# tensorlink-lab/tensorlink

Measured on AMD Instinct MI355X. Metric: output tokens/sec (Qwen2.5-7B serving, PP sharded), higher is better.
Workload: dtype bf16; 1 GPU; model=Qwen/Qwen2.5-7B-Instruct, global_batch=256, seq_len=512, parallelism=pp1, micro_batches=4

## Files before the change

tensorlink_amd/models/dense.py:

```python

from __future__ import annotations

import dataclasses

import math
from typing import List, Optional

import torch
import torch.nn as nn

from tensorlink_amd import ops
from tensorlink_amd.models.configs import ModelConfig


class KVCache:

    def __init__(self, n_layers: int, batch: int, max_seq: int, config,
                 device, dtype=torch.bfloat16):
        self.k = [torch.zeros(batch, config.num_key_value_heads, max_seq,
                              config.head_dim, device=device, dtype=dtype)
                  for _ in range(n_layers)]
        self.v = [torch.zeros_like(self.k[0]) for _ in range(n_layers)]
        self.seq_lens = torch.zeros(batch, device=device, dtype=torch.int32)
        self.max_seq = max_seq
# ... 79 lines not shown
        eps = self.config.rms_norm_eps
        fuse = fuse and kv_cache is not None and not training
        if fuse and not self.use_qk_norm:
            qkv = _project(self.qkv_proj, x, allow_bias=True)
        else:
            qkv = self.qkv_proj(x)
        flat_pos = positions.reshape(-1)

        if training or kv_cache is None:
            q, k, v = self._split_qkv(qkv, B, S)
            if self.use_qk_norm:
                q = ops.rmsnorm(q.contiguous(), self.q_norm.to(q.dtype), eps)
                k = ops.rmsnorm(k.contiguous(), self.k_norm.to(k.dtype), eps)
            if training:
                q2, k2 = ops.apply_rope(q.reshape(B * S, self.n_heads, -1),
                                        k.reshape(B * S, self.n_kv, -1),
                                        flat_pos, self.inv_freq)
                q = q2.view(B, S, self.n_heads, -1)
                k = k2.view(B, S, self.n_kv, -1)
                out = ops.attention_train(q, k, v, causal=True,
                                          scale=self.scale)
            else:
                q = q.contiguous()
                k = k.contiguous()
                ops.apply_rope_(q.view(B * S, self.n_heads, -1),
                                k.view(B * S, self.n_kv, -1), flat_pos,
                                self.inv_freq)
                out = ops.attention_prefill(q, k, v.contiguous(),
                                            causal=True, scale=self.scale)
            return self.o_proj(out.reshape(B, S, -1))

        table = getattr(kv_cache, "table", None)
        if self.use_qk_norm:
            q, k, v = self._split_qkv(qkv, B, S)
            q = ops.rmsnorm(q.contiguous(), self.q_norm.to(q.dtype), eps)
            k = ops.rmsnorm(k.contiguous(), self.k_norm.to(k.dtype), eps)
            qkv = torch.cat([q.reshape(B, S, -1), k.reshape(B, S, -1),
                             v.reshape(B, S, -1)], dim=-1)
        if not isinstance(qkv, ops.Partials):
            qkv = qkv.reshape(B * S, -1)
        q = ops.rope_append_(qkv, kv_cache.k[layer_idx],
                             kv_cache.v[layer_idx], flat_pos, self.inv_freq,
                             S, self.n_heads, self.n_kv, block_table=table)
        q = q.view(B, S, self.n_heads, self.head_dim)
        if S == 1 and fuse:
            out = ops.attention_decode(
                q, kv_cache.k[layer_idx], kv_cache.v[layer_idx],
                kv_cache.seq_lens, scale=self.scale, block_table=table,
                len_add=1)
        elif S == 1:
            out = ops.attention_decode(
                q, kv_cache.k[layer_idx], kv_cache.v[layer_idx],
                kv_cache.seq_lens + 1, scale=self.scale, block_table=table)
        else:
            if B > 1:
                assert int(kv_cache.seq_lens.min()) == \
                    int(kv_cache.seq_lens.max()), \
                    "ragged cached prefill needs per-row q_off"
            off = int(kv_cache.seq_lens.max())
            kv_len = off + S
            if table is None:
                k_attn = kv_cache.k[layer_idx][:, :, :kv_len].permute(
                    0, 2, 1, 3).contiguous()
                v_attn = kv_cache.v[layer_idx][:, :, :kv_len].permute(
                    0, 2, 1, 3).contiguous()
            else:
                k_attn, v_attn = kv_cache.gather_contiguous(layer_idx, kv_len)
            out = ops.attention_prefill(q, k_attn, v_attn, causal=True,
                                        scale=self.scale, q_off=off)
        if fuse:
            return _project(self.o_proj, out.reshape(B, S, -1))
        return self.o_proj(out.reshape(B, S, -1))


class MLP(nn.Module):
    def __init__(self, config: ModelConfig):
        super().__init__()
        h, i = config.hidden_size, config.intermediate_size
        self.inter = i
        self.gate_up_proj = TLLinear(h, 2 * i, bias=False)
        self.down_proj = TLLinear(i, h, bias=False)

    def forward(self, x, fuse: bool = False):
        gu = self.gate_up_proj(x)
        if torch.is_grad_enabled() and gu.requires_grad:
            gate, up = gu.split([self.inter, self.inter], dim=-1)
            return self.down_proj(ops.swiglu(gate.contiguous(),
                                             up.contiguous()))
        if fuse:
            return _project(self.down_proj, ops.swiglu_fused(gu))
        return self.down_proj(ops.swiglu_fused(gu))


class MoEMLP(nn.Module):

    def __init__(self, config: ModelConfig):
        super().__init__()
        h, i = config.hidden_size, config.intermediate_size
        self.num_experts = config.num_local_experts
        self.top_k = config.num_experts_per_tok
        self.gate = nn.Linear(h, self.num_experts, bias=False)
        expert_cfg = (config if config.expert_intermediate_size == i
                      else dataclasses.replace(
                          config,
                          intermediate_size=config.expert_intermediate_size))
        self.experts = nn.ModuleList([MLP(expert_cfg)
                                      for _ in range(self.num_experts)])

    def _fused_kind(self):
        from tensorlink_amd.models.quant import Fp4Linear, Fp8Linear
        e0 = self.experts[0]
        if isinstance(e0.gate_up_proj, Fp8Linear):
            return "fp8"
        if isinstance(e0.gate_up_proj, Fp4Linear):
            for e in self.experts:
                for p in (e.gate_up_proj, e.down_proj):
                    if not (isinstance(p, Fp4Linear) and p.bias is None
                            and p.out_features % 64 == 0
                            and p.in_features % 128 == 0):
                        return None
            return "fp4"
        if isinstance(e0.gate_up_proj, nn.Linear) \
                and e0.gate_up_proj.bias is None:
            return "bf16"
        return None

    def _tables(self, dev, kind):
        wname = {"fp8": "weight_fp8", "fp4": "packed"}.get(kind, "weight")
        sname = {"fp8": "scale", "fp4": "exponents"}.get(kind)
        gus = [getattr(e.gate_up_proj, wname) for e in self.experts]
        key = (str(dev), kind, gus[0].data_ptr())
        if getattr(self, "_tbl_key", None) != key:
            downs = [getattr(e.down_proj, wname) for e in self.experts]

            def mk(ts):
                if kind == "fp4":
                    assert all(t.is_contiguous()
                               and t.data_ptr() % 16 == 0 for t in ts), \
                        "fp4 expert tensors must be contiguous and " \
                        "16-byte aligned"
                return torch.tensor([t.data_ptr() for t in ts],
                                    dtype=torch.int64, device=dev)
            self._gu_ptrs = mk(gus)
            self._down_ptrs = mk(downs)
            if sname is not None:
                self._gu_scales = mk([getattr(e.gate_up_proj, sname)
                                      for e in self.experts])
                self._down_scales = mk([getattr(e.down_proj, sname)
                                        for e in self.experts])
            else:
                self._gu_scales = self._down_scales = None
            self._tbl_key = key
        return (self._gu_ptrs, self._down_ptrs, self._gu_scales,
                self._down_scales)

    def _fused_forward(self, flat, rw, idx, kind=None):
        C = ops._require_ext()
        kind = kind if kind is not None else self._fused_kind()
        E, k = self.num_experts, self.top_k
        T, H = flat.shape
        P = T * k
        dev = flat.device
        gu_p, down_p, gu_s, down_s = self._tables(dev, kind)
        fi = idx.reshape(-1)
        order = fi.argsort(stable=True)
        counts = torch.zeros(E, device=dev, dtype=torch.long)
        counts.scatter_add_(0, fi, torch.ones_like(fi))
        seg = torch.zeros(E + 1, device=dev, dtype=torch.int32)
        seg[1:] = counts.cumsum(0)
        pair_tok = (order // k).to(torch.int32)
        Ie = self.experts[0].inter
        if kind == "fp4":
            gu = ops.mxfp4_moe_gemm(flat.contiguous(), pair_tok, seg, gu_p,
                                    gu_s, 2 * Ie)
# ... 186 lines not shown
```

tensorlink_amd/ops/__init__.py:

```python

from __future__ import annotations

import math
from typing import Optional

import torch

from tensorlink_amd.ops import reference as ref

_C = None
_IMPORT_ERROR: Optional[BaseException] = None
try:
    from tensorlink_amd import _C
except Exception as e:
    _IMPORT_ERROR = e


def extension_loaded() -> bool:
    return _C is not None


def _require_ext():
    if _C is None:
        raise RuntimeError(
# ... 234 lines not shown
        ctx.causal = causal
        ctx.scale = scale
        return out

    @staticmethod
    def backward(ctx, dout):
        C = _require_ext()
        q, k, v, out, lse = ctx.saved_tensors
        delta = (dout.float() * out.float()).sum(-1)
        delta = delta.permute(0, 2, 1).contiguous()
        dq, dk, dv = C.attn_bwd(q.contiguous(), k.contiguous(),
                                v.contiguous(), dout.contiguous(), lse,
                                delta, ctx.scale, ctx.causal)
        return dq, dk, dv, None, None


def attention_train(q, k, v, causal: bool = True,
                    scale: Optional[float] = None) -> torch.Tensor:
    B, S, Hq, D = q.shape
    Hkv = k.shape[2]
    if scale is None:
        scale = 1.0 / math.sqrt(D)
    if (q.is_cuda and q.dtype == torch.bfloat16 and _C is not None
            and D in (64, 128) and k.shape[1] == S):
        return _FlashAttnFn.apply(q, k, v, causal, scale)
    qt = q.transpose(1, 2)
    kt = k.transpose(1, 2)
    vt = v.transpose(1, 2)
    try:
        out = torch.nn.functional.scaled_dot_product_attention(
            qt, kt, vt, is_causal=causal, scale=scale, enable_gqa=True)
    except (TypeError, RuntimeError):
        rep = Hq // Hkv
        out = torch.nn.functional.scaled_dot_product_attention(
            qt, kt.repeat_interleave(rep, dim=1),
            vt.repeat_interleave(rep, dim=1), is_causal=causal, scale=scale)
    return out.transpose(1, 2)


def attention_decode(q, k_cache, v_cache, seq_lens,
                     scale: Optional[float] = None, n_split: int = 0,
                     block_table: Optional[torch.Tensor] = None,
                     len_add: int = 0) -> torch.Tensor:
    squeeze = q.dim() == 4
    if squeeze:
        q3 = q.squeeze(1)
    else:
        q3 = q
    scale = scale if scale is not None else 1.0 / math.sqrt(q3.shape[-1])
    if not _on_gpu(q3):
        if len_add:
            seq_lens = seq_lens + len_add
        if block_table is not None:
            B = q3.shape[0]
            L = int(seq_lens.max())
            np_ = (L + 127) // 128
            idx = block_table[:, :np_].long()
            kc = k_cache[idx].permute(0, 1, 3, 2, 4)
            vc = v_cache[idx].permute(0, 1, 3, 2, 4)
            kc = kc.reshape(B, np_ * 128, *kc.shape[3:])[:, :L]
            vc = vc.reshape(B, np_ * 128, *vc.shape[3:])[:, :L]
            out = ref.attention_decode(q3.unsqueeze(1), kc, vc, seq_lens,
                                       scale)
        else:
            out = ref.attention_decode(q3.unsqueeze(1),
                                       k_cache.permute(0, 2, 1, 3),
                                       v_cache.permute(0, 2, 1, 3),
                                       seq_lens, scale)
        return out if squeeze else out.squeeze(1)
    out = _require_ext().decode_attn(
        q3.contiguous(), k_cache, v_cache, seq_lens.int(), scale, n_split,
        block_table.int() if block_table is not None else None, len_add)
    return out.unsqueeze(1) if squeeze else out


import os as _os

GEMM_M_MAX = int(_os.environ.get("TL_GEMM_M_MAX", "512"))

gemm_dispatch_count = 0


_LIB_CLASSES = frozenset(
    c for c in _os.environ.get("TL_GEMM_LIB_CLASSES",
                               "gateup").split(",") if c)


def _gemm_class(N: int, K: int) -> str:
    if N >= 65536:
        return "wide"
    if N >= 16384:
        return "gateup"
    if K >= 8192:
        return "deepk"
    return "narrow"


def _use_tl_gemm(M: int, N: int, K: int) -> bool:
    return (K % 32 == 0 and N % 64 == 0 and M <= GEMM_M_MAX
            and _gemm_class(N, K) not in _LIB_CLASSES)


def linear(x: torch.Tensor, weight: torch.Tensor,
           bias: Optional[torch.Tensor] = None) -> torch.Tensor:
    global gemm_dispatch_count
    if (x.is_cuda and not torch.is_grad_enabled()
            and x.dtype == torch.bfloat16
            and not _os.environ.get("TL_NO_SKINNY")):
        K = x.shape[-1]
        M = x.numel() // K
        N = weight.shape[0]
        if _use_tl_gemm(M, N, K):
            gemm_dispatch_count += 1
            return _require_ext().skinny_gemm(
                x.contiguous(), weight,
                bias.to(torch.bfloat16) if bias is not None else None)
    return torch.nn.functional.linear(x, weight, bias)


def decode_fusion_enabled() -> bool:
    return not _os.environ.get("TL_NO_DECODE_FUSION")


def linear_partials(x: torch.Tensor, weight: torch.Tensor,
                    bias: Optional[torch.Tensor] = None):
    global gemm_dispatch_count
    if (x.is_cuda and not torch.is_grad_enabled()
            and x.dtype == torch.bfloat16
            and not _os.environ.get("TL_NO_SKINNY")):
        K = x.shape[-1]
        M = x.numel() // K
        N = weight.shape[0]
        if _use_tl_gemm(M, N, K):
            gemm_dispatch_count += 1
            b = bias.to(torch.bfloat16) if bias is not None else None
            out = _require_ext().skinny_gemm_partials(x.contiguous(),
                                                      weight, b)
            if out.dtype == torch.float32:
                return Partials(out, b)
            return out
    return linear(x, weight, bias)


mxfp4_dispatch_count = 0


def _use_mxfp4_gemm(M: int, N: int, K: int) -> bool:
    return (N > 0 and N % 64 == 0 and K > 0 and K % 128 == 0
            and 1 <= M <= min(GEMM_M_MAX, 512))


def mxfp4_linear(x: torch.Tensor, packed: torch.Tensor,
                 exponents: torch.Tensor,
                 bias: Optional[torch.Tensor] = None) -> torch.Tensor:
    global mxfp4_dispatch_count
    if not _on_gpu(x):
        return ref.mxfp4_linear(x, packed, exponents, bias)
    K = x.shape[-1]
    M = x.numel() // K if K else 0
    N = packed.shape[0]
    if (x.dtype == torch.bfloat16 and _C is not None
            and _use_mxfp4_gemm(M, N, K)):
        mxfp4_dispatch_count += 1
        return _C.mxfp4_gemm(
            x.contiguous(), packed.contiguous(), exponents.contiguous(),
            bias.to(torch.bfloat16).contiguous()
            if bias is not None else None)
    w = ref.dequantize_mxfp4(packed, exponents, dtype=torch.bfloat16)
    return torch.nn.functional.linear(
        x, w.to(x.dtype), bias.to(x.dtype) if bias is not None else None)


mxfp4_moe_dispatch_count = 0


def mxfp4_moe_gemm(x: torch.Tensor, tok_idx: Optional[torch.Tensor],
                   seg_off: torch.Tensor, p_ptrs: torch.Tensor,
                   e_ptrs: torch.Tensor, N: int) -> torch.Tensor:
    global mxfp4_moe_dispatch_count
    out = _require_ext().mxfp4_moe_gemm(x, tok_idx, seg_off, p_ptrs, e_ptrs,
                                        N)
    mxfp4_moe_dispatch_count += 1
    return out


def adamw_(param: torch.Tensor, grad: torch.Tensor, exp_avg: torch.Tensor,
           exp_avg_sq: torch.Tensor, *, lr: float, beta1: float = 0.9,
           beta2: float = 0.999, eps: float = 1e-8,
           weight_decay: float = 0.0, step: int = 1) -> None:
    if not _on_gpu(param):
        ref.adamw_step(param, grad, exp_avg, exp_avg_sq, lr=lr, beta1=beta1,
                       beta2=beta2, eps=eps, weight_decay=weight_decay,
                       step=step)
        return
    _require_ext().adamw_(param, grad.contiguous(), exp_avg, exp_avg_sq, lr,
                          beta1, beta2, eps, weight_decay, step)


def _splitmix64(x: int) -> int:
    x = (x + 0x9E3779B97F4A7C15) & (2 ** 64 - 1)
# ... 37 lines not shown
```

tensorlink_amd/ops/csrc/bindings.cpp:

```cpp

#include <torch/extension.h>

#include <c10/hip/HIPStream.h>
#include <hip/hip_runtime.h>

extern "C" {
void tl_rmsnorm_fwd(const void* x, const void* residual, const void* w,
                    void* y, void* r_out, void* rstd, int64_t N, int H,
                    float eps, hipStream_t stream);
void tl_rmsnorm_add_fwd(const void* x, const void* residual, const void* w,
                        void* y, void* r_out, int64_t N, int H, float eps,
                        int n_split, int mode, hipStream_t stream);
void tl_rmsnorm_bwd(const void* dy, const void* x, const void* w,
                    const void* rstd, void* dx, void* dw, void* dw_partial,
                    int n_blocks, int64_t N, int H, hipStream_t stream);
void tl_rope(void* q, void* k, const void* positions, const void* inv_freq,
             int64_t T, int Hq, int Hkv, int D, float sign,
             hipStream_t stream);
void tl_swiglu_fwd(const void* gate, const void* up, void* out, int64_t n,
                   hipStream_t stream);
void tl_swiglu_bwd(const void* dout, const void* gate, const void* up,
                   void* dgate, void* dup, int64_t n, hipStream_t stream);
void tl_adamw(void* param, const void* grad, void* m, void* v, int64_t n,
              int is_bf16, float lr, double beta1, double beta2, float eps,
              float weight_decay, int step, hipStream_t stream);
void tl_decode_attn(const void* q, const void* k_cache, const void* v_cache,
                    const void* seq_lens, void* out, int B, int Hq, int Hkv,
                    int Smax, int D, float scale, int len_add,
                    hipStream_t stream);
void tl_prefill_attn(const void* q, const void* k, const void* v, void* out,
                     int B, int Sq, int Skv, int q_off, int Hq, int Hkv,
                     int D, float scale, int causal, hipStream_t stream);
void tl_rope_append(const void* qkv, const void* bias, void* q_out,
                    void* k_cache, void* v_cache, const void* positions,
                    const void* inv_freq, const void* block_table,
                    int64_t T, int row_stride, int S, int Hq, int Hkv,
                    int D, int Smax, int bt_stride, int n_split,
                    int inv_bf16, hipStream_t stream);
void tl_swiglu_fused(const void* gu, void* out, int64_t N, int I,
                     hipStream_t stream);
void tl_decode_attn_mfma(const void* q, const void* k_cache,
                         const void* v_cache, const void* seq_lens,
                         const void* block_table, void* out,
                         void* partial, void* partial_ml, int B, int Hq,
                         int Hkv, int Smax, int D, float scale, int n_split,
                         int bt_stride, int per_row, int len_add,
                         hipStream_t stream);
void tl_skinny_gemm(const void* x, const void* w, const void* bias,
                    void* out, void* partial, int M, int N, int K,
                    int n_split, hipStream_t stream);
void tl_gemm_tiled(const void* x, const void* w, const void* bias, void* out,
                   void* partial, int M, int N, int K, int n_split,
                   hipStream_t stream);
void tl_skinny_gemm_partials(const void* x, const void* w, const void* bias,
                             void* out, void* partial, int M, int N, int K,
                             int n_split, hipStream_t stream);
void tl_gemm_tiled_partials(const void* x, const void* w, const void* bias,
                            void* out, void* partial, int M, int N, int K,
                            int n_split, hipStream_t stream);
void tl_sample(const void* logits, const void* temps, const void* top_ps,
               const void* top_ks, const void* pres, const void* freqs,
               void* counts, const void* seeds, const void* ctr, void* out,
               uint64_t seed_base, int B, int V, hipStream_t stream);
void tl_bump_counter(void* ctr, hipStream_t stream);
void tl_moe_gemm(const void* x, const void* tok_idx, const void* seg_off,
                 const void* w_ptrs, const void* s_ptrs, void* out, int E,
                 int N, int K, int fp8, hipStream_t stream);
void tl_mxfp4_gemm(const void* x, const void* packed, const void* exps,
                   const void* bias, void* out, void* partial, int M, int N,
                   int K, int n_split, hipStream_t stream);
void tl_mxfp4_moe_gemm(const void* x, const void* tok_idx,
                       const void* seg_off, const void* p_ptrs,
                       const void* e_ptrs, void* out, void* partial, int T,
                       int P, int E, int N, int K, int n_split,
                       hipStream_t stream);
void tl_prefill_attn_lse(const void* q, const void* k, const void* v,
                         void* out, void* lse, int B, int Sq, int Skv,
                         int q_off, int Hq, int Hkv, int D, float scale,
                         int causal, hipStream_t stream);
void tl_attn_bwd(const void* q, const void* k, const void* v,
                 const void* dout, const void* lse, const void* delta,
                 void* dq, void* dk, void* dv, int B, int S, int Hq,
                 int Hkv, int D, float scale, int causal,
                 hipStream_t stream);
}

namespace {

hipStream_t cur_stream() {
  return c10::hip::getCurrentHIPStream().stream();
}

int tl_split_for_len(int L) {
  int ns = 1;
  while (ns < 16 && L > 1024 * ns) ns <<= 1;
  return ns;
}

#define CHECK_IN(t, d)                                              \
  TORCH_CHECK((t).is_cuda(), #t " must be on GPU");                 \
  TORCH_CHECK((t).is_contiguous(), #t " must be contiguous");       \
  TORCH_CHECK((t).scalar_type() == (d), #t " wrong dtype")

using torch::Tensor;

std::vector<Tensor> rmsnorm_fwd(Tensor x, c10::optional<Tensor> residual,
                                Tensor w, double eps, bool save_rstd) {
  CHECK_IN(x, torch::kBFloat16);
  CHECK_IN(w, torch::kBFloat16);
  const int H = x.size(-1);
  TORCH_CHECK(H % 8 == 0, "H must be divisible by 8");
  TORCH_CHECK(H <= 16384, "rmsnorm supports H <= 16384");
  const int64_t N = x.numel() / H;
  auto y = torch::empty_like(x);
  Tensor rstd, r_out;
  if (save_rstd) rstd = torch::empty({N}, x.options().dtype(torch::kFloat));
  const void* res_ptr = nullptr;
  void* rout_ptr = nullptr;
  if (residual.has_value()) {
    CHECK_IN(residual.value(), torch::kBFloat16);
    r_out = torch::empty_like(x);
    res_ptr = residual->data_ptr();
    rout_ptr = r_out.data_ptr();
  }
  tl_rmsnorm_fwd(x.data_ptr(), res_ptr, w.data_ptr(), y.data_ptr(), rout_ptr,
                 save_rstd ? rstd.data_ptr() : nullptr, N, H, (float)eps,
                 cur_stream());
  std::vector<Tensor> outs = {y};
  if (residual.has_value()) outs.push_back(r_out);
  if (save_rstd) outs.push_back(rstd);
  return outs;
}

std::vector<Tensor> rmsnorm_add_fwd(Tensor x, Tensor residual,
                                    c10::optional<Tensor> w, double eps,
                                    int64_t mode) {
  CHECK_IN(residual, torch::kBFloat16);
  TORCH_CHECK(mode >= 1 && mode <= 3, "mode must be 1, 2 or 3");
  const int H = residual.size(-1);
  TORCH_CHECK(H % 8 == 0, "H must be divisible by 8");
  TORCH_CHECK(H <= 16384, "rmsnorm supports H <= 16384");
  const int64_t N = residual.numel() / H;
// ... 281 lines not shown
}

static int gemm_split_target() {
  static int t = [] {
    const char* e = getenv("TL_GEMM_SPLIT_TARGET");
    return e ? atoi(e) : 256;
  }();
  return t;
}

static int gemm_n_split(int N, int K) {
  if (N >= 65536) {
    int n_split = 1;
    while (((N + 255) / 256) * n_split < gemm_split_target() &&
           n_split < 16 && (K / 64) / (n_split * 2) >= 16)
      n_split <<= 1;
    return n_split;
  }
  int n_split = 1;
  while ((N / 64) * n_split < gemm_split_target() && n_split < 8 &&
         (K / 32) / (n_split * 2) >= 2)
    n_split <<= 1;
  return n_split;
}

Tensor skinny_gemm(Tensor x, Tensor w, c10::optional<Tensor> bias) {
  CHECK_IN(x, torch::kBFloat16);
  CHECK_IN(w, torch::kBFloat16);
  const int K = x.size(-1);
  const int64_t M = x.numel() / K;
  const int N = w.size(0);
  TORCH_CHECK(w.size(1) == K, "K mismatch");
  TORCH_CHECK(K % 32 == 0 && N % 64 == 0, "unsupported shape");
  auto sizes = x.sizes().vec();
  sizes.back() = N;
  auto out = torch::empty(sizes, x.options());
  const void* bp = nullptr;
  if (bias.has_value()) {
    CHECK_IN(bias.value(), torch::kBFloat16);
    bp = bias->data_ptr();
  }
  const int n_split = gemm_n_split(N, K);
  Tensor partial;
  void* pp = nullptr;
  if (n_split > 1) {
    partial = torch::empty({(int64_t)n_split * M * N},
                           x.options().dtype(torch::kFloat));
    pp = partial.data_ptr();
  }
  if (M <= 64)
    tl_skinny_gemm(x.data_ptr(), w.data_ptr(), bp, out.data_ptr(), pp,
                   (int)M, N, K, n_split, cur_stream());
  else
    tl_gemm_tiled(x.data_ptr(), w.data_ptr(), bp, out.data_ptr(), pp,
                  (int)M, N, K, n_split, cur_stream());
  return out;
}

Tensor skinny_gemm_partials(Tensor x, Tensor w, c10::optional<Tensor> bias) {
  CHECK_IN(x, torch::kBFloat16);
  CHECK_IN(w, torch::kBFloat16);
  const int K = x.size(-1);
  const int64_t M = x.numel() / K;
  const int N = w.size(0);
  TORCH_CHECK(w.size(1) == K, "K mismatch");
  TORCH_CHECK(K % 32 == 0 && N % 64 == 0, "unsupported shape");
  const int n_split = gemm_n_split(N, K);
  if (n_split == 1) return skinny_gemm(x, w, bias);
  auto sizes = x.sizes().vec();
  sizes.back() = N;
  sizes.insert(sizes.begin(), n_split);
  auto partial = torch::empty(sizes, x.options().dtype(torch::kFloat));
  if (M <= 64)
    tl_skinny_gemm_partials(x.data_ptr(), w.data_ptr(), nullptr, nullptr,
                            partial.data_ptr(), (int)M, N, K, n_split,
                            cur_stream());
  else
    tl_gemm_tiled_partials(x.data_ptr(), w.data_ptr(), nullptr, nullptr,
                           partial.data_ptr(), (int)M, N, K, n_split,
                           cur_stream());
  return partial;
}

static int mxfp4_split_for_blocks(int blocks, int K) {
  int n_split = 1;
  while (blocks * n_split < 256 && n_split < 8 &&
         (K / 128) / (n_split * 2) >= 2)
    n_split <<= 1;
  return n_split;
}

static int mxfp4_n_split(int N, int K) {
  return mxfp4_split_for_blocks(N / 64, K);
}

static int mxfp4_moe_n_split(int N, int K, int E) {
  return mxfp4_split_for_blocks((N / 64) * E, K);
}

int64_t mxfp4_n_split_py(int64_t N, int64_t K) {
  TORCH_CHECK(N > 0 && K > 0 && N % 64 == 0 && K % 128 == 0,
              "unsupported shape");
  return mxfp4_n_split((int)N, (int)K);
}

int64_t mxfp4_moe_n_split_py(int64_t N, int64_t K, int64_t E) {
  TORCH_CHECK(N > 0 && K > 0 && E > 0 && N % 64 == 0 && K % 128 == 0,
              "unsupported shape");
  return mxfp4_moe_n_split((int)N, (int)K, (int)E);
}

Tensor mxfp4_gemm(Tensor x, Tensor packed, Tensor exponents,
                  c10::optional<Tensor> bias) {
  CHECK_IN(x, torch::kBFloat16);
  CHECK_IN(packed, torch::kByte);
  CHECK_IN(exponents, torch::kChar);
  TORCH_CHECK(packed.dim() == 2 && exponents.dim() == 2,
              "packed / exponents must be 2-D");
  TORCH_CHECK(x.dim() >= 1, "x must have a K dimension");
  const int64_t K = x.size(-1);
  const int64_t N = packed.size(0);
  TORCH_CHECK(K > 0 && N > 0 && N % 64 == 0 && K % 128 == 0,
              "unsupported shape: need N % 64 == 0 and K % 128 == 0");
  TORCH_CHECK(packed.size(1) * 2 == K, "packed must be [N, K/2]");
  TORCH_CHECK(exponents.size(0) == N && exponents.size(1) * 32 == K,
              "exponents must be [N, K/32]");
  const int64_t M = x.numel() / K;
  TORCH_CHECK(M >= 1 && M <= 512, "mxfp4_gemm supports 1 <= M <= 512");
  TORCH_CHECK(packed.device() == x.device() &&
                  exponents.device() == x.device(),
              "operands must share a device");
  auto sizes = x.sizes().vec();
  sizes.back() = N;
  auto out = torch::empty(sizes, x.options());
  const void* bp = nullptr;
  if (bias.has_value()) {
    CHECK_IN(bias.value(), torch::kBFloat16);
    TORCH_CHECK(bias->numel() == N, "bias must be [N]");
    bp = bias->data_ptr();
  }
  const int n_split = mxfp4_n_split((int)N, (int)K);
  Tensor partial;
  void* pp = nullptr;
  if (n_split > 1) {
    partial = torch::empty({(int64_t)n_split * M * N},
                           x.options().dtype(torch::kFloat));
    pp = partial.data_ptr();
  }
  tl_mxfp4_gemm(x.data_ptr(), packed.data_ptr(), exponents.data_ptr(), bp,
                out.data_ptr(), pp, (int)M, (int)N, (int)K, n_split,
                cur_stream());
  return out;
}

Tensor sample_tokens(Tensor logits, Tensor temps, Tensor top_ps,
                     Tensor top_ks, Tensor pres, Tensor freqs,
                     c10::optional<Tensor> counts,
                     c10::optional<Tensor> seeds,
                     c10::optional<Tensor> counter, int64_t seed_base) {
  CHECK_IN(logits, torch::kBFloat16);
  CHECK_IN(temps, torch::kFloat);
  CHECK_IN(top_ps, torch::kFloat);
  CHECK_IN(top_ks, torch::kInt);
  CHECK_IN(pres, torch::kFloat);
  CHECK_IN(freqs, torch::kFloat);
  const int B = logits.size(0);
// ... 40 lines not shown
  const void* ti = nullptr;
  int64_t P;
  if (tok_idx.has_value()) {
    CHECK_IN(tok_idx.value(), torch::kInt);
    ti = tok_idx->data_ptr();
    P = tok_idx->size(0);
  } else {
    P = x.size(0);
  }
  const void* sp = nullptr;
  if (fp8) {
    TORCH_CHECK(s_ptrs.has_value(), "fp8 needs scale pointers");
    CHECK_IN(s_ptrs.value(), torch::kLong);
    sp = s_ptrs->data_ptr();
  }
  auto out = torch::empty({P, N}, x.options());
  tl_moe_gemm(x.data_ptr(), ti, seg_off.data_ptr(), w_ptrs.data_ptr(), sp,
              out.data_ptr(), E, (int)N, K, fp8 ? 1 : 0, cur_stream());
  return out;
}

Tensor mxfp4_moe_gemm(Tensor x, c10::optional<Tensor> tok_idx,
                      Tensor seg_off, Tensor p_ptrs, Tensor e_ptrs,
                      int64_t N, int64_t n_split_override) {
  CHECK_IN(x, torch::kBFloat16);
  CHECK_IN(seg_off, torch::kInt);
  CHECK_IN(p_ptrs, torch::kLong);
  CHECK_IN(e_ptrs, torch::kLong);
  TORCH_CHECK(x.dim() == 2, "x must be [T, K]");
  const int64_t T = x.size(0);
  const int64_t K = x.size(1);
  TORCH_CHECK(K > 0 && N > 0 && N % 64 == 0 && K % 128 == 0,
              "unsupported shape: need N % 64 == 0 and K % 128 == 0");
  TORCH_CHECK(p_ptrs.dim() == 1 && e_ptrs.dim() == 1 &&
                  p_ptrs.size(0) == e_ptrs.size(0),
              "pointer tables must both be [E]");
  const int64_t E = p_ptrs.size(0);
  TORCH_CHECK(E >= 1 && E <= 65535, "need 1 <= E <= 65535");
  TORCH_CHECK(seg_off.dim() == 1 && seg_off.size(0) == E + 1,
              "seg_off must be [E+1]");
  TORCH_CHECK(seg_off.device() == x.device() &&
                  p_ptrs.device() == x.device() &&
                  e_ptrs.device() == x.device(),
              "operands must share a device");
  const void* ti = nullptr;
  int64_t P = T;
  if (tok_idx.has_value()) {
    CHECK_IN(tok_idx.value(), torch::kInt);
    TORCH_CHECK(tok_idx->dim() == 1, "tok_idx must be [P]");
    TORCH_CHECK(tok_idx->device() == x.device(),
                "operands must share a device");
    ti = tok_idx->data_ptr();
    P = tok_idx->size(0);
  }
  TORCH_CHECK(P * N < (int64_t)1 << 31 && T * K < (int64_t)1 << 40,
              "mxfp4_moe_gemm: call too large");
  auto out = torch::empty({P, N}, x.options());
  if (P == 0) return out;
  TORCH_CHECK(T >= 1, "x has no rows");
  const int n_split = n_split_override > 0
                          ? (int)n_split_override
                          : mxfp4_moe_n_split((int)N, (int)K, (int)E);
  TORCH_CHECK(n_split >= 1 && n_split <= 8, "bad split count");
  Tensor partial;
  void* pp = nullptr;
  if (n_split > 1) {
    partial = torch::empty({(int64_t)n_split * P * N},
                           x.options().dtype(torch::kFloat));
    pp = partial.data_ptr();
  }
  tl_mxfp4_moe_gemm(x.data_ptr(), ti, seg_off.data_ptr(), p_ptrs.data_ptr(),
                    e_ptrs.data_ptr(), out.data_ptr(), pp, (int)T, (int)P,
                    (int)E, (int)N, (int)K, n_split, cur_stream());
  return out;
}

}

PYBIND11_MODULE(TORCH_EXTENSION_NAME, mod) {
  mod.def("rope_append_", &rope_append_,
          "fused RoPE + KV-cache append from fused-QKV rows");
  mod.def("swiglu_fused", &swiglu_fused, "silu-mul on fused [.,2I] rows");
  mod.def("skinny_gemm", &skinny_gemm, "decode-M GEMM: x @ W^T + bias");
  mod.def("skinny_gemm_partials", &skinny_gemm_partials,
          "decode-M GEMM handing out its fp32 split-K partials");
  mod.def("rmsnorm_add_fwd", &rmsnorm_add_fwd,
          "residual add + RMSNorm from bf16 or split-K partials");
  mod.def("rmsnorm_fwd", &rmsnorm_fwd, "fused RMSNorm fwd (+residual)");
  mod.def("rmsnorm_bwd", &rmsnorm_bwd, "RMSNorm bwd");
  mod.def("rope_", &rope_, "in-place RoPE apply");
  mod.def("swiglu_fwd", &swiglu_fwd, "silu(gate)*up");
  mod.def("swiglu_bwd", &swiglu_bwd, "SwiGLU bwd");
  mod.def("adamw_", &adamw_, "fused AdamW step");
  mod.def("decode_attn", &decode_attn, "GQA decode attention over KV cache");
  mod.def("prefill_attn", &prefill_attn, "causal GQA prefill attention");
  mod.def("sample_tokens", &sample_tokens,
          "fused penalties/temperature/top-k/top-p sampling, one block/row");
  mod.def("bump_sample_counter", &bump_sample_counter,
          "advance the graph-safe sampling RNG counter");
  mod.def("moe_gemm", &moe_gemm,
          "grouped expert GEMM over expert-sorted pair rows");
  mod.def("mxfp4_gemm", &mxfp4_gemm,
          "weight-only MXFP4 GEMM: x @ dequant(packed, exponents)^T + bias");
  mod.def("mxfp4_n_split", &mxfp4_n_split_py,
          "split-K count of mxfp4_gemm for (N, K)");
  mod.def("mxfp4_moe_gemm", &mxfp4_moe_gemm,
          "grouped MXFP4 expert GEMM over expert-sorted pair rows",
          pybind11::arg("x"), pybind11::arg("tok_idx"),
          pybind11::arg("seg_off"), pybind11::arg("p_ptrs"),
          pybind11::arg("e_ptrs"), pybind11::arg("N"),
          pybind11::arg("n_split_override") = 0);
  mod.def("mxfp4_moe_n_split", &mxfp4_moe_n_split_py,
          "split-K count of mxfp4_moe_gemm for (N, K, E)");
  mod.def("prefill_attn_lse", &prefill_attn_lse,
          "causal GQA prefill attention returning (out, logsumexp)");
  mod.def("attn_bwd", &attn_bwd,
          "flash-attention backward: (dq, dk, dv) from saved lse/delta");
}
```

tensorlink_amd/ops/csrc/swiglu.hip:

```cpp

#include "common.hpp"

namespace {

constexpr int BLOCK = 256;

DEVINLINE float silu(float x) { return x / (1.f + __expf(-x)); }

__global__ __launch_bounds__(BLOCK) void swiglu_fwd_kernel(
    const bf16* __restrict__ gate, const bf16* __restrict__ up,
    bf16* __restrict__ out, int64_t n8) {
  const int64_t i = ((int64_t)blockIdx.x * BLOCK + threadIdx.x);
  if (i >= n8) return;
  bf16x8 g = reinterpret_cast<const bf16x8*>(gate)[i];
  bf16x8 u = reinterpret_cast<const bf16x8*>(up)[i];
  bf16x8 o;
#pragma unroll
  for (int j = 0; j < 8; ++j)
    o.v[j] = f2bf(silu(bf2f(g.v[j])) * bf2f(u.v[j]));
  reinterpret_cast<bf16x8*>(out)[i] = o;
}

__global__ __launch_bounds__(BLOCK) void swiglu_fused_kernel(
    const bf16* __restrict__ gu, bf16* __restrict__ out, int64_t N, int I) {
  const int64_t i = ((int64_t)blockIdx.x * BLOCK + threadIdx.x) * 8;
  if (i >= N * (int64_t)I) return;
  const int64_t r = i / I;
  const int64_t c = i - r * I;
  const bf16x8 g = *reinterpret_cast<const bf16x8*>(gu + r * 2 * I + c);
  const bf16x8 u = *reinterpret_cast<const bf16x8*>(gu + r * 2 * I + I + c);
  bf16x8 o;
#pragma unroll
  for (int j = 0; j < 8; ++j)
    o.v[j] = f2bf(silu(bf2f(g.v[j])) * bf2f(u.v[j]));
  *reinterpret_cast<bf16x8*>(out + r * I + c) = o;
}

__global__ __launch_bounds__(BLOCK) void swiglu_bwd_kernel(
    const bf16* __restrict__ dout, const bf16* __restrict__ gate,
    const bf16* __restrict__ up, bf16* __restrict__ dgate,
    bf16* __restrict__ dup, int64_t n8) {
  const int64_t i = ((int64_t)blockIdx.x * BLOCK + threadIdx.x);
  if (i >= n8) return;
  bf16x8 dO = reinterpret_cast<const bf16x8*>(dout)[i];
  bf16x8 g = reinterpret_cast<const bf16x8*>(gate)[i];
  bf16x8 u = reinterpret_cast<const bf16x8*>(up)[i];
  bf16x8 dg, du;
#pragma unroll
  for (int j = 0; j < 8; ++j) {
    const float gv = bf2f(g.v[j]);
    const float sig = 1.f / (1.f + __expf(-gv));
    const float si = gv * sig;
    const float dsilu = sig * (1.f + gv * (1.f - sig));
    const float dov = bf2f(dO.v[j]);
    dg.v[j] = f2bf(dov * bf2f(u.v[j]) * dsilu);
    du.v[j] = f2bf(dov * si);
  }
  reinterpret_cast<bf16x8*>(dgate)[i] = dg;
  reinterpret_cast<bf16x8*>(dup)[i] = du;
}

}

extern "C" {

void tl_swiglu_fwd(const void* gate, const void* up, void* out, int64_t n,
                   hipStream_t stream) {
  const int64_t n8 = n / 8;
  dim3 grid((uint32_t)cdiv(n8, BLOCK)), block(BLOCK);
  hipLaunchKernelGGL(swiglu_fwd_kernel, grid, block, 0, stream,
                     (const bf16*)gate, (const bf16*)up, (bf16*)out, n8);
}

void tl_swiglu_fused(const void* gu, void* out, int64_t N, int I,
                     hipStream_t stream) {
  const int64_t work = N * (int64_t)I / 8;
  dim3 grid((uint32_t)((work + BLOCK - 1) / BLOCK)), block(BLOCK);
  hipLaunchKernelGGL(swiglu_fused_kernel, grid, block, 0, stream,
                     (const bf16*)gu, (bf16*)out, N, I);
}

void tl_swiglu_bwd(const void* dout, const void* gate, const void* up,
                   void* dgate, void* dup, int64_t n, hipStream_t stream) {
  const int64_t n8 = n / 8;
  dim3 grid((uint32_t)cdiv(n8, BLOCK)), block(BLOCK);
  hipLaunchKernelGGL(swiglu_bwd_kernel, grid, block, 0, stream,
                     (const bf16*)dout, (const bf16*)gate, (const bf16*)up,
                     (bf16*)dgate, (bf16*)dup, n8);
}

}
```

Before: 13800 tokens/s.

## Add column-balanced gate_up GEMM with fused SwiGLU epilogue

```diff
diff --git a/tensorlink_amd/models/dense.py b/tensorlink_amd/models/dense.py
--- a/tensorlink_amd/models/dense.py
+++ b/tensorlink_amd/models/dense.py
@@ -185,14 +185,19 @@
         self.down_proj = TLLinear(i, h, bias=False)
 
     def forward(self, x, fuse: bool = False):
-        gu = self.gate_up_proj(x)
-        if torch.is_grad_enabled() and gu.requires_grad:
-            gate, up = gu.split([self.inter, self.inter], dim=-1)
-            return self.down_proj(ops.swiglu(gate.contiguous(),
-                                             up.contiguous()))
+        if (type(self.gate_up_proj) is TLLinear and not
+                torch.is_grad_enabled()):
+            act = ops.gate_up_swiglu(x, self.gate_up_proj.weight)
+        else:
+            gu = self.gate_up_proj(x)
+            if torch.is_grad_enabled() and gu.requires_grad:
+                gate, up = gu.split([self.inter, self.inter], dim=-1)
+                return self.down_proj(ops.swiglu(gate.contiguous(),
+                                                 up.contiguous()))
+            act = ops.swiglu_fused(gu)
         if fuse:
-            return _project(self.down_proj, ops.swiglu_fused(gu))
-        return self.down_proj(ops.swiglu_fused(gu))
+            return _project(self.down_proj, act)
+        return self.down_proj(act)
 
 
 class MoEMLP(nn.Module):
diff --git a/tensorlink_amd/ops/__init__.py b/tensorlink_amd/ops/__init__.py
--- a/tensorlink_amd/ops/__init__.py
+++ b/tensorlink_amd/ops/__init__.py
@@ -340,8 +340,7 @@
 
 
 _LIB_CLASSES = frozenset(
-    c for c in _os.environ.get("TL_GEMM_LIB_CLASSES",
-                               "gateup").split(",") if c)
+    c for c in _os.environ.get("TL_GEMM_LIB_CLASSES", "").split(",") if c)
 
 
 def _gemm_class(N: int, K: int) -> str:
@@ -359,21 +358,53 @@
             and _gemm_class(N, K) not in _LIB_CLASSES)
 
 
+_n_split_cache = {}
+
+
+def _use_colbal(M: int, N: int, K: int) -> bool:
+    if not (65 <= M and _use_tl_gemm(M, N, K)
+            and _gemm_class(N, K) == "gateup"
+            and not _os.environ.get("TL_NO_COLBAL")):
+        return False
+    ns = _n_split_cache.get((N, K))
+    if ns is None:
+        ns = _n_split_cache[(N, K)] = _require_ext().gemm_n_split(N, K)
+    return ns == 1
+
+
+def _family_input(x: torch.Tensor) -> bool:
+    return (x.is_cuda and not torch.is_grad_enabled()
+            and x.dtype == torch.bfloat16
+            and not _os.environ.get("TL_NO_SKINNY"))
+
+
 def linear(x: torch.Tensor, weight: torch.Tensor,
            bias: Optional[torch.Tensor] = None) -> torch.Tensor:
     global gemm_dispatch_count
-    if (x.is_cuda and not torch.is_grad_enabled()
-            and x.dtype == torch.bfloat16
-            and not _os.environ.get("TL_NO_SKINNY")):
+    if _family_input(x):
         K = x.shape[-1]
         M = x.numel() // K
         N = weight.shape[0]
+        if bias is None and _use_colbal(M, N, K):
+            gemm_dispatch_count += 1
+            return _require_ext().gemm_colbal(x.contiguous(), weight)
         if _use_tl_gemm(M, N, K):
             gemm_dispatch_count += 1
             return _require_ext().skinny_gemm(
                 x.contiguous(), weight,
                 bias.to(torch.bfloat16) if bias is not None else None)
     return torch.nn.functional.linear(x, weight, bias)
+
+
+def gate_up_swiglu(x: torch.Tensor, weight: torch.Tensor) -> torch.Tensor:
+    global gemm_dispatch_count
+    if _family_input(x) and not _os.environ.get("TL_NO_GATEUP_FUSION"):
+        K = x.shape[-1]
+        M = x.numel() // K
+        if _use_colbal(M, weight.shape[0], K):
+            gemm_dispatch_count += 1
+            return _require_ext().gemm_colbal_swiglu(x.contiguous(), weight)
+    return swiglu_fused(linear(x, weight))
 
 
 def decode_fusion_enabled() -> bool:
diff --git a/tensorlink_amd/ops/csrc/bindings.cpp b/tensorlink_amd/ops/csrc/bindings.cpp
--- a/tensorlink_amd/ops/csrc/bindings.cpp
+++ b/tensorlink_amd/ops/csrc/bindings.cpp
@@ -58,6 +58,8 @@
 void tl_gemm_tiled_partials(const void* x, const void* w, const void* bias,
                             void* out, void* partial, int M, int N, int K,
                             int n_split, hipStream_t stream);
+void tl_gemm_colbal(const void* x, const void* w, void* out, int M, int N,
+                    int K, int n_blocks, int fused, hipStream_t stream);
 void tl_sample(const void* logits, const void* temps, const void* top_ps,
                const void* top_ks, const void* pres, const void* freqs,
                void* counts, const void* seeds, const void* ctr, void* out,
@@ -505,6 +507,52 @@
   return partial;
 }
 
+static int device_cu_count(int dev) {
+  static int cus[64] = {0};
+  TORCH_CHECK(dev >= 0 && dev < 64, "device index out of range");
+  if (cus[dev] == 0) {
+    int n = 0;
+    TORCH_CHECK(hipDeviceGetAttribute(
+                    &n, hipDeviceAttributeMultiprocessorCount, dev) ==
+                        hipSuccess && n > 0,
+                "cannot read the CU count");
+    cus[dev] = n;
+  }
+  return cus[dev];
+}
+
+static Tensor gemm_colbal_impl(Tensor x, Tensor w, int64_t n_blocks,
+                               bool fused) {
+  CHECK_IN(x, torch::kBFloat16);
+  CHECK_IN(w, torch::kBFloat16);
+  const int K = x.size(-1);
+  const int64_t M = x.numel() / K;
+  const int N = w.size(0);
+  TORCH_CHECK(w.dim() == 2 && w.size(1) == K, "K mismatch");
+  TORCH_CHECK(K % 32 == 0 && K >= 32 && M >= 1 && M < (1 << 24),
+              "unsupported shape");
+  TORCH_CHECK(N % (fused ? 32 : 16) == 0 && N > 0, "unsupported width");
+  TORCH_CHECK(gemm_n_split(N, K) == 1,
+              "gemm_colbal serves only shapes the policy does not split");
+  if (n_blocks <= 0) n_blocks = device_cu_count(x.get_device());
+  TORCH_CHECK(n_blocks <= 65535, "n_blocks too large");
+  const int NO = fused ? N / 2 : N;
+  auto sizes = x.sizes().vec();
+  sizes.back() = NO;
+  auto out = torch::empty(sizes, x.options());
+  tl_gemm_colbal(x.data_ptr(), w.data_ptr(), out.data_ptr(), (int)M, NO, K,
+                 (int)n_blocks, fused ? 1 : 0, cur_stream());
+  return out;
+}
+
+Tensor gemm_colbal(Tensor x, Tensor w, int64_t n_blocks) {
+  return gemm_colbal_impl(x, w, n_blocks, false);
+}
+
+Tensor gemm_colbal_swiglu(Tensor x, Tensor w_gate_up, int64_t n_blocks) {
+  return gemm_colbal_impl(x, w_gate_up, n_blocks, true);
+}
+
 static int mxfp4_split_for_blocks(int blocks, int K) {
   int n_split = 1;
   while (blocks * n_split < 256 && n_split < 8 &&
@@ -711,6 +759,14 @@
           "fused RoPE + KV-cache append from fused-QKV rows");
   mod.def("swiglu_fused", &swiglu_fused, "silu-mul on fused [.,2I] rows");
   mod.def("skinny_gemm", &skinny_gemm, "decode-M GEMM: x @ W^T + bias");
+  mod.def("gemm_n_split", &gemm_n_split,
+          "split-K count the GEMM family's (N,K)-only policy gives");
+  mod.def("gemm_colbal", &gemm_colbal,
+          "column-balanced one-pass GEMM: x @ W^T (n_split == 1 shapes)",
+          py::arg("x"), py::arg("w"), py::arg("n_blocks") = 0);
+  mod.def("gemm_colbal_swiglu", &gemm_colbal_swiglu,
+          "column-balanced gate_up GEMM with SwiGLU on the accumulators",
+          py::arg("x"), py::arg("w_gate_up"), py::arg("n_blocks") = 0);
   mod.def("skinny_gemm_partials", &skinny_gemm_partials,
           "decode-M GEMM handing out its fp32 split-K partials");
   mod.def("rmsnorm_add_fwd", &rmsnorm_add_fwd,
diff --git a/tensorlink_amd/ops/csrc/gemm_colbal.hip b/tensorlink_amd/ops/csrc/gemm_colbal.hip
--- /dev/null
+++ b/tensorlink_amd/ops/csrc/gemm_colbal.hip
@@ -0,0 +1,241 @@
+
+#include "common.hpp"
+#include "swiglu_common.hpp"
+
+namespace {
+
+using f32x4 = __attribute__((ext_vector_type(4))) float;
+typedef __bf16 bf16x8_t __attribute__((ext_vector_type(8)));
+
+constexpr int CB_BM = 256;
+constexpr int CB_SLOTS = 10;
+constexpr int CB_ROWS = CB_BM + CB_SLOTS * 16;
+constexpr int CB_STAGES = 3;
+constexpr int CB_STAGE_ELEMS = CB_ROWS * 64;
+constexpr int CB_CPAD = 168;
+
+template <int N>
+DEVINLINE void cb_waitcnt_vm() {
+  asm volatile("s_waitcnt vmcnt(%0)" ::"n"(N) : "memory");
+}
+
+template <int FUSED>
+__global__ __launch_bounds__(512, 1) void gemm_colbal_kernel(
+    const bf16* __restrict__ x,
+    const bf16* __restrict__ w,
+    bf16* __restrict__ out,
+    int M, int NO, int K) {
+  const int tid = threadIdx.x;
+  const int lane = tid & 63;
+  const int wave = __builtin_amdgcn_readfirstlane(tid >> 6);
+  const int col = lane & 15;
+  const int quad = lane >> 4;
+  const int wm = wave >> 1;
+  const int wn = wave & 1;
+  const int l8 = lane >> 3, c8 = lane & 7;
+  const int m_base = blockIdx.z * CB_BM;
+
+  constexpr int SPT = FUSED ? 2 : 1;
+  constexpr int MAXT = CB_SLOTS / SPT;
+
+  const int T = NO / 16, G = gridDim.x, b = blockIdx.x;
+  const int q = T / G, r = T % G;
+  const int cnt = q + (b < r ? 1 : 0);
+  const int start = b * q + min(b, r);
+  if (cnt == 0) return;
+  const int n_sub = (cnt + MAXT - 1) / MAXT;
+
+  __shared__ bf16 lds[CB_STAGES * CB_STAGE_ELEMS];
+
+  const bool active = m_base + wm * 64 < M;
+  const int n_full = K / 64, n_chunks = (K + 63) / 64;
+
+  for (int s = 0; s < n_sub; ++s) {
+    const int sq = cnt / n_sub, sr = cnt % n_sub;
+    const int t0 = start + s * sq + min(s, sr);
+    const int tc = sq + (s < sr ? 1 : 0);
+
+    int64_t xoff[4], woff[3];
+#pragma unroll
+    for (int g = 0; g < 4; ++g) {
+      const int row = (wave * 4 + g) * 8 + l8;
+      xoff[g] = (int64_t)min(m_base + row, M - 1) * K;
+    }
+#pragma unroll
+    for (int g = 0; g < 3; ++g) {
+      const int wchunk = min(wave + g * 8, 19);
+      const int slot = wchunk >> 1;
+      const int half = FUSED ? (slot >= MAXT ? 1 : 0) : 0;
+      const int tile = t0 + min(slot - half * MAXT, tc - 1);
+      woff[g] = ((int64_t)half * NO + tile * 16 + (wchunk & 1) * 8 + l8) * K;
+    }
+
+    auto stage = [&](int bufi, int k0) {
+      bf16* sbase = lds + bufi * CB_STAGE_ELEMS;
+      const int kc = min(k0 + (c8 ^ l8) * 8, K - 8);
+#pragma unroll
+      for (int g = 0; g < 4; ++g) {
+        auto gsrc = (const __attribute__((address_space(1))) void*)(
+            x + xoff[g] + kc);
+        auto ldst = (__attribute__((address_space(3))) void*)(
+            sbase + (wave * 4 + g) * 8 * 64);
+        __builtin_amdgcn_global_load_lds(gsrc, ldst, 16, 0, 0);
+      }
+#pragma unroll
+      for (int g = 0; g < 3; ++g) {
+        if (g == 2 && wave >= 4) break;
+        auto gsrc = (const __attribute__((address_space(1))) void*)(
+            w + woff[g] + kc);
+        auto ldst = (__attribute__((address_space(3))) void*)(
+            sbase + (CB_BM + (wave + g * 8) * 8) * 64);
+        __builtin_amdgcn_global_load_lds(gsrc, ldst, 16, 0, 0);
+      }
+    };
+
+    f32x4 acc[20];
+#pragma unroll
+    for (int i = 0; i < 20; ++i) acc[i] = (f32x4){0.f, 0.f, 0.f, 0.f};
+
+    const bf16* sb = lds;
+    bf16x8_t bfrag[2][5], afrag[2][4];
+    auto read_frags = [&](int kk) {
+#pragma unroll
+      for (int nt = 0; nt < 5; ++nt) {
+        const int wrow = (wn * 5 + nt) * 16 + col;
+        const int wslot = (kk * 4 + quad) ^ (wrow & 7);
+        bfrag[kk][nt] = *reinterpret_cast<const bf16x8_t*>(
+            sb + (CB_BM + wrow) * 64 + wslot * 8);
+      }
+#pragma unroll
+      for (int mt = 0; mt < 4; ++mt) {
+        const int row = wm * 64 + mt * 16 + col;
+        const int slot = (kk * 4 + quad) ^ (row & 7);
+        afrag[kk][mt] = *reinterpret_cast<const bf16x8_t*>(
+            sb + row * 64 + slot * 8);
+      }
+    };
+    auto mfmas = [&](int kk) {
+#pragma unroll
+      for (int mt = 0; mt < 4; ++mt)
+#pragma unroll
+        for (int nt = 0; nt < 5; ++nt)
+          acc[mt * 5 + nt] = __builtin_amdgcn_mfma_f32_16x16x32_bf16(
+              afrag[kk][mt], bfrag[kk][nt], acc[mt * 5 + nt], 0, 0, 0);
+    };
+    auto retire = [&](int t) {
+      if (t + 1 < n_chunks) {
+        if (wave < 4) cb_waitcnt_vm<7>();
+        else cb_waitcnt_vm<6>();
+      } else {
+        cb_waitcnt_vm<0>();
+      }
+      asm volatile("s_waitcnt lgkmcnt(0)" ::: "memory");
+      __builtin_amdgcn_s_barrier();
+    };
+
+#define CB_INTERLEAVE()                                                     \
+  _Pragma("unroll") for (int i = 0; i < 9; ++i) {                           \
+    __builtin_amdgcn_sched_group_barrier(0x008, 1, 0);          \
+    __builtin_amdgcn_sched_group_barrier(0x100, 1, 0);       \
+  }                                                                         \
+  __builtin_amdgcn_sched_group_barrier(0x008, 11, 0)
+
+    stage(0, 0);
+    if (n_chunks > 1) stage(1, 64);
+    retire(0);
+    if (n_chunks > 2) stage(2, 128);
+    int cur = 0;
+    if (active) read_frags(0);
+    const int n_piped = min(n_full, n_chunks - 1);
+    for (int t = 0; t < n_piped; ++t) {
+      if (active) {
+        __builtin_amdgcn_sched_barrier(0);
+        __builtin_amdgcn_s_setprio(1);
+        read_frags(1);
+        mfmas(0);
+        CB_INTERLEAVE();
+        __builtin_amdgcn_sched_barrier(0);
+        __builtin_amdgcn_s_setprio(0);
+      }
+      retire(t + 1);
+      if (t + 3 < n_chunks) stage(cur, (t + 3) * 64);
+      cur = cur == 2 ? 0 : cur + 1;
+      if (active) {
+        sb = lds + cur * CB_STAGE_ELEMS;
+        __builtin_amdgcn_sched_barrier(0);
+        __builtin_amdgcn_s_setprio(1);
+        read_frags(0);
+        mfmas(1);
+        CB_INTERLEAVE();
+        __builtin_amdgcn_sched_barrier(0);
+        __builtin_amdgcn_s_setprio(0);
+      }
+    }
+    if (active) {
+      __builtin_amdgcn_sched_barrier(0);
+      __builtin_amdgcn_s_setprio(1);
+      read_frags(1);
+      mfmas(0);
+      CB_INTERLEAVE();
+      __builtin_amdgcn_sched_barrier(0);
+      if (n_chunks == n_full) mfmas(1);
+      __builtin_amdgcn_s_setprio(0);
+    }
+#undef CB_INTERLEAVE
+
+    asm volatile("s_waitcnt lgkmcnt(0)" ::: "memory");
+    __syncthreads();
+    int etid = tid;
+    asm volatile("" : "+v"(etid));
+    const int ecol = etid & 15, equad = (etid >> 4) & 3;
+#pragma unroll
+    for (int mt = 0; mt < 4; ++mt)
+#pragma unroll
+      for (int nt = 0; nt < 5; ++nt)
+#pragma unroll
+        for (int i = 0; i < 4; ++i) {
+          const int row = wm * 64 + mt * 16 + equad * 4 + i;
+          const int c = (wn * 5 + nt) * 16 + ecol;
+          lds[row * CB_CPAD + c] = f2bf(acc[mt * 5 + nt][i] + 0.f);
+        }
+    __syncthreads();
+
+    constexpr int VPR = 2 * MAXT;
+#pragma unroll
+    for (int it = 0; it < CB_BM * VPR / 512; ++it) {
+      const int v = it * 512 + etid;
+      const int row = v / VPR, cv = v % VPR;
+      const int orow = m_base + row;
+      if (cv < tc * 2 && orow < M) {
+        bf16x8 o = *reinterpret_cast<const bf16x8*>(
+            &lds[row * CB_CPAD + cv * 8]);
+        if (FUSED) {
+          const bf16x8 u = *reinterpret_cast<const bf16x8*>(
+              &lds[row * CB_CPAD + MAXT * 16 + cv * 8]);
+#pragma unroll
+          for (int j = 0; j < 8; ++j) o.v[j] = swiglu_bf16(o.v[j], u.v[j]);
+        }
+        *reinterpret_cast<bf16x8*>(
+            out + (int64_t)orow * NO + t0 * 16 + cv * 8) = o;
+      }
+    }
+    __syncthreads();
+  }
+}
+
+}
+
+extern "C" {
+
+void tl_gemm_colbal(const void* x, const void* w, void* out, int M, int N,
+                    int K, int n_blocks, int fused, hipStream_t stream) {
+  dim3 grid(n_blocks, 1, cdiv(M, CB_BM)), block(512);
+  if (fused)
+    hipLaunchKernelGGL((gemm_colbal_kernel<1>), grid, block, 0, stream,
+                       (const bf16*)x, (const bf16*)w, (bf16*)out, M, N, K);
+  else
+    hipLaunchKernelGGL((gemm_colbal_kernel<0>), grid, block, 0, stream,
+                       (const bf16*)x, (const bf16*)w, (bf16*)out, M, N, K);
+}
+
+}
diff --git a/tensorlink_amd/ops/csrc/swiglu.hip b/tensorlink_amd/ops/csrc/swiglu.hip
--- a/tensorlink_amd/ops/csrc/swiglu.hip
+++ b/tensorlink_amd/ops/csrc/swiglu.hip
@@ -1,11 +1,10 @@
 
 #include "common.hpp"
+#include "swiglu_common.hpp"
 
 namespace {
 
 constexpr int BLOCK = 256;
-
-DEVINLINE float silu(float x) { return x / (1.f + __expf(-x)); }
 
 __global__ __launch_bounds__(BLOCK) void swiglu_fwd_kernel(
     const bf16* __restrict__ gate, const bf16* __restrict__ up,
@@ -17,7 +16,7 @@
   bf16x8 o;
 #pragma unroll
   for (int j = 0; j < 8; ++j)
-    o.v[j] = f2bf(silu(bf2f(g.v[j])) * bf2f(u.v[j]));
+    o.v[j] = swiglu_bf16(g.v[j], u.v[j]);
   reinterpret_cast<bf16x8*>(out)[i] = o;
 }
 
@@ -32,7 +31,7 @@
   bf16x8 o;
 #pragma unroll
   for (int j = 0; j < 8; ++j)
-    o.v[j] = f2bf(silu(bf2f(g.v[j])) * bf2f(u.v[j]));
+    o.v[j] = swiglu_bf16(g.v[j], u.v[j]);
   *reinterpret_cast<bf16x8*>(out + r * I + c) = o;
 }
 
diff --git a/tensorlink_amd/ops/csrc/swiglu_common.hpp b/tensorlink_amd/ops/csrc/swiglu_common.hpp
--- /dev/null
+++ b/tensorlink_amd/ops/csrc/swiglu_common.hpp
@@ -0,0 +1,9 @@
+#pragma once
+
+#include "common.hpp"
+
+DEVINLINE float silu(float x) { return x / (1.f + __expf(-x)); }
+
+DEVINLINE bf16 swiglu_bf16(bf16 g, bf16 u) {
+  return f2bf(silu(bf2f(g)) * bf2f(u));
+}
```

Result: faster. 14090 tokens/s, median of 6 (+2.1%).
